# kikimo/tla-raft

Measured on AMD Instinct MI355X. Metric: distinct states/sec (whole node) + wall-time to exhaust, higher is better.
Workload: dtype u32

## Files before the change

tla-raft_amd/csrc/rmc_engine.hip:

```cpp
#include <hip/hip_runtime.h>
#include <hipcub/hipcub.hpp>

#include <algorithm>
#include <array>
#include <chrono>
#include <condition_variable>
#include <cstdio>
#include <cstdlib>
#include <cstring>
#include <memory>
#include <mutex>
#include <set>
#include <string>
#include <thread>
#include <vector>

#include <fcntl.h>
#include <sys/mman.h>
#include <unistd.h>

#include "rmc.h"
#include "rmc_kernels.h"
#include "rmc_plan.h"
#include "rmc_graph.h"
// ... 727 lines not shown
    void graph_level(Shard &s, uint64_t gid_cur, uint64_t n_par, uint64_t gid_nxt, uint64_t n_new, uint64_t bound_pos,
                     uint32_t bound_key, int kind) {
        try {
            graph_states(s, s.nxt_off, s.nbase(), n_new, gid_nxt);
            graph_edges(s, gid_cur, n_par, bound_pos, bound_key, kind);
        } catch (const Fail &e) {
            finished = true;
            status = e.code;
            throw;
        }
    }

    bool inited = false, finished = false;
    bool device_released = false;
    int status = RMC_OK;
    int depth = 0;
    uint64_t total_generated = 0, total_distinct = 0, queue_at_end = 0;
    int violated = -1;
    uint64_t err_ref = 0;
    uint32_t err_last_slot = KEY_NONE;
    std::vector<uint64_t> glevel;
    int L_shard = 0;
    std::vector<TraceStep> trace;
    double seconds = 0;

    KParams base(const Shard &s) const {
        KParams P{};
        P.d = U.d;
        P.E = cfg.max_election;
        P.R = cfg.max_restart;
        P.seeded = cfg.spec_variant == RMC_SPEC_SEEDED;
        P.quirks = (cfg.spec_variant == RMC_SPEC_SPLIT_BRAIN ? 1u : 0u) | (cfg.spec_variant == RMC_SPEC_COMMIT_PAST_LOG ? 2u : 0u);
        P.check_deadlock = cfg.check_deadlock;
        P.inv_mask = cfg.invariants;
        P.inv_order = inv_order;
        P.t.info = d_info;
        P.t.nat2id = d_nat2id;
        P.t.gmsg = d_gmsg;
        P.t.seeds = d_seeds;
        P.t.np = np;
        P.t.bmw = (uint32_t)((U.info.size() + 31) / 32);
        P.seen = s.seen();
        P.rcap = ~0ull;
        P.err = s.err;
        P.flags = s.flags;
        P.par = s.par;
        P.pslot = s.pslot;
        P.trace_base = s.tdev;
        return P;
    }

    void ring_params(const Shard &s, KParams &P) const {
        P.front = s.R;
        P.foff = s.cur_off;
        P.fbase = s.cur_wbase;
        P.rcap = s.rcap;
        P.next = s.R;
        P.noff = s.nxt_off;
        P.nbase = s.nbase();
    }

    KParams chunk_params(const Shard &s) const {
        KParams Q = base(s);
        ring_params(s, Q);
        Q.cnt = s.cnt; Q.fp = s.fp; Q.wpos = s.wpos; Q.wcnt = s.wcnt; Q.wacc = s.wacc; Q.pnm = s.pnm;
        Q.wposw = s.wposw; Q.bw = s.bw; Q.bg = s.bg; Q.boff = s.boff; Q.bww = s.bww; Q.boffw = s.boffw;
        Q.bn = s.bn; Q.boffn = s.boffn;
        Q.tickets = s.tickets; Q.ctick = s.ctick; Q.sum = s.sum;
        Q.score = s.score; Q.lslot = s.lslot; Q.ET = s.E; Q.hctx = s.hctx;
        return Q;
    }

    const int lookahead = env_int("RMC_LOOKAHEAD", 1, 0, 1);
    bool two_sets() const { return lookahead && !multi; }

    static uint32_t probe_dedup_entries() {
        const int v = env_int("RMC_PROBE_DEDUP", 1, 0, (int)PD_ENTRIES);
        if (v <= 1) return v ? PD_ENTRIES : 0u;
        uint32_t n = 2;
        while (2 * n <= (uint32_t)v) n *= 2;
        return n;
    }
    const uint32_t probe_dedup = probe_dedup_entries();
    const uint32_t probe_run = (uint32_t)env_int("RMC_PROBE_RUN", 0, 0, 64);
    const int probe_log = env_int("RMC_PROBE_DEDUP_LOG", 0, 0, 1);

    static constexpr unsigned ITEMS_MIN_BLOCKS = 2048;
    const int items_grid_env = env_int("RMC_ITEMS_GRID", 0, 0, 1 << 20);
    unsigned items_xgrid = 0, items_cgrid = 0;
    void size_items_grids(int cus) {
        int xb = 0, cb = 0;
        HIPCHK(ks.items_blocks(&xb, &cb));
        auto whole = [&](int per_cu) {
            const unsigned gen = (unsigned)(per_cu * cus);
            return gen ? (ITEMS_MIN_BLOCKS + gen - 1) / gen * gen : 0u;
        };
        items_xgrid = items_grid_env ? (unsigned)items_grid_env : whole(xb);
        items_cgrid = items_grid_env ? (unsigned)items_grid_env : whole(cb);
    }

    void swap_staging(Shard &s) {
        Staging &a = s.alt;
        std::swap(s.score, a.score); std::swap(s.hctx, a.hctx); std::swap(s.cnt, a.cnt); std::swap(s.pnm, a.pnm);
        std::swap(s.hcnt, a.hcnt); std::swap(s.hoff, a.hoff);
        std::swap(s.err, a.err); std::swap(s.sum, a.sum); std::swap(s.flags, a.flags);
        std::swap(s.xdone, a.done); std::swap(s.xt0, a.t0); std::swap(s.xt1, a.t1); std::swap(s.xtimed, a.timed);
        s.ocnt = reinterpret_cast<uint32_t *>(s.sum + SUM_OCNT);
    }
    static void alt_params(const Staging &a, KParams &Q) {
        Q.score = a.score; Q.hctx = a.hctx; Q.cnt = a.cnt; Q.pnm = a.pnm;
        Q.err = a.err; Q.sum = a.sum; Q.flags = a.flags;
    }
    void xwait() {
        if (xpending) HIPCHK(hipStreamSynchronize(xstream));
    }
    void drop_lookahead() {
        if (!xpending) return;
        xpending = false;
// ... 3762 lines not shown
```

tla-raft_amd/csrc/rmc_kernels.h:

```cpp
#pragma once
#include <hip/hip_runtime.h>
#include <stdint.h>

#include "rmc_spec.h"

namespace rmc {

struct Tables {
    const uint32_t *info;
    const uint16_t *nat2id;
    const ulonglong2 *gmsg;
    const uint64_t *seeds;
    int np;
    uint32_t bmw;
};

struct ESlot {
    unsigned long long x, y;
    unsigned long long k;
    unsigned long long pad;
};

struct Seen {
    ulonglong2 *T;
// ... 7 lines not shown
enum CtlStop : uint32_t { CTL_RUN = 0, CTL_DONE = 1, CTL_ERROR = 2, CTL_HOST = 3 };
struct LevelCtl {
    unsigned long long cur_n;
    unsigned long long gid_cur;
    unsigned long long T_count;
    unsigned long long Lmask;
    unsigned long long cur_wbase, cur_words;
    unsigned long long off_cap, rcap, trace_base, trace_cap, T_cap, chunk_parents, Lcap_max;
    uint32_t level;
    uint32_t epoch;
    uint32_t stop;
    uint32_t done_levels;
    uint32_t batch;
    uint32_t pad_;
};
struct LevelRec { unsigned long long expanded, generated, new_states, words, self_loops; };
constexpr int LREC_CAP = 1024;
struct HostLoop {
    uint32_t done;
    uint32_t stop;
    uint32_t pad_[2];
    LevelCtl ctl;
    LevelRec rec[LREC_CAP];
};
constexpr uint32_t WTILE = 1024;
constexpr uint32_t WTILES_MAX = 4096;
constexpr int SUM_WORDS = 7;
constexpr int SUM_INS = 9;
constexpr int SUM_INS_COMMIT = 10;
constexpr int SUM_NZ = 16;
constexpr int SUM_SELF = 17;
constexpr int SUM_HFP = 18;
constexpr uint32_t PD_ENTRIES = 512;
constexpr int PROBE_RUN = 2;
constexpr int SUM_OCNT = 20;
constexpr int SUM_PDROP = 56;
constexpr int SUM_SELF_STRIPE = 64, SELF_STRIDE = 16, SELF_STRIPES = 8;
constexpr int SUM_WORDS_TOTAL = 192;


struct KParams {
    Dims d;
    int E, R, seeded, check_deadlock;
    uint32_t inv_mask;
    uint32_t inv_order;
    Tables t;
    const uint32_t *front;
    const uint64_t *foff;
    uint64_t fbase, rcap;
    uint64_t p_begin, p_end;
    uint32_t *cnt;
    uint32_t *hcnt;
    uint32_t *hoff;
    const uint32_t *off;
    ulonglong2 *fp;
    const uint32_t *wflag;
    uint32_t *wpos;
    Seen seen;
    uint32_t *next;
    uint64_t *noff;
    uint64_t nbase;
    uint64_t next_wbase;
    uint64_t next_base;
    uint64_t *par;
    uint16_t *pslot;
    uint64_t trace_base;
    uint64_t gid_next_base;
    uint64_t gid_parent_base;
    unsigned long long *err;
    uint32_t *flags;
    int route;
    uint4 *xside;
    uint32_t *ocnt;
    uint32_t nown;
    ESlot *OT;
    uint64_t ot_mask, gblk;
    uint32_t ot_round, self;
    int split;
    uint32_t *hctx;
    uint32_t pdedup, prun;
    uint32_t quirks;
    uint4 *score;
    uint32_t *lslot;
    ESlot *ET;
    uint64_t Lmask;
    uint32_t epoch;
    uint32_t *wcnt;
    uint32_t *wacc;
    uint32_t *pnm;
    uint32_t *wposw;
    uint32_t *bw, *bg, *boff;
    uint32_t *bww, *boffw;
    uint32_t *bn, *boffn;
    uint32_t *plist;
    uint32_t *tickets;
    uint32_t *ctick;
    unsigned long long *sum;
    LevelCtl *ctl;
    LevelCtl *ctl_next;
    LevelRec *lrec;
    HostLoop *hloop;
    uint32_t done_levels;
    uint32_t *out_keys;
    uint32_t *out_count;
};

enum WalkEnd : uint32_t {
    WALK_DEPTH = 0,
    WALK_STUCK = 1,
    WALK_DEADLOCK = 2,
    WALK_ASSERT = 3,
    WALK_VIOLATION = 4,
    WALK_EVAL = 5,
// ... 108 lines not shown
```

tla-raft_amd/csrc/rmc_kernels.hip:

```cpp
#include <hip/hip_runtime.h>

#include <algorithm>

#include "rmc_kernels.h"

#ifdef RMC_PHASE_PROF
__device__ unsigned long long g_phase[16];
#define PHASE_DECL unsigned long long _acc[8] = {0, 0, 0, 0, 0, 0, 0, 0}; long long _tp = clock64();
#define PHASE(k) do { const long long _t = clock64(); _acc[k] += (unsigned long long)(_t - _tp); _tp = _t; } while (0)
#define PHASE_FLUSH_AT(b) do { if (threadIdx.x == 0) for (int _k = 0; _k < 8; _k++) atomicAdd(&g_phase[(b) + _k], _acc[_k]); } while (0)
#define PHASE_FLUSH PHASE_FLUSH_AT(0)
extern "C" int rmc_debug_phases(unsigned long long *out, int reset) {
    if (hipMemcpyFromSymbol(out, HIP_SYMBOL(g_phase), sizeof(unsigned long long) * 16) != hipSuccess) return -1;
    if (reset) {
        unsigned long long z[16] = {0};
        if (hipMemcpyToSymbol(HIP_SYMBOL(g_phase), z, sizeof(z)) != hipSuccess) return -1;
    }
    return 16;
}
#else
#define PHASE_DECL
#define PHASE(k) do {} while (0)
#define PHASE_FLUSH do {} while (0)
#define PHASE_FLUSH_AT(b) do {} while (0)
#endif

#ifndef RMC_N3_WAVES
#define RMC_N3_WAVES 4
#endif
#ifndef RMC_N3_COMMIT_WAVES
#define RMC_N3_COMMIT_WAVES 1
#endif
#ifndef RMC_GRID_PER_CU
#define RMC_GRID_PER_CU 32
#endif
#ifndef RMC_WIDE_WAVES
#define RMC_WIDE_WAVES 2
#endif

namespace rmc {

enum Mode { M_SINGLE = 3, M_FUSED = 4 };

template <int N>
__device__ __forceinline__ uint32_t sel(const uint32_t *a, int i) {
    uint32_t r = a[0];
#pragma unroll
    for (int k = 1; k < N; k++) r = (i == k) ? a[k] : r;
    return r;
}

__device__ __forceinline__ uint32_t rdlane(uint32_t v, int l) { return __builtin_amdgcn_readlane(v, l); }
__device__ __forceinline__ uint64_t rdlane64(uint64_t v, int l) {
    uint32_t lo = __builtin_amdgcn_readlane((uint32_t)v, l);
    uint32_t hi = __builtin_amdgcn_readlane((uint32_t)(v >> 32), l);
    return ((uint64_t)hi << 32) | lo;
}
// ... 1537 lines not shown
    return vf | (ct << 4) | (role << 8) | (ci << 12) | (ll << 16) | (s << 20);
}

template <int MCAP>
__device__ __forceinline__ bool ids_contain(const uint16_t *ids, uint32_t nm, uint32_t g) {
    uint32_t pos = 0;
#pragma unroll
    for (uint32_t st = (uint32_t)MCAP; st; st >>= 1)
        if (pos + st <= nm && (uint32_t)ids[pos + st - 1] < g) pos += st;
    return pos < nm && (uint32_t)ids[pos] == g;
}

template <int NADD>
struct RowSucc {
    uint32_t w0, lw, mirow, nirow, pend, misc;
    uint32_t key;
    uint32_t nadd;
    uint32_t add[NADD];
    uint32_t ainf[NADD];
    bool self;
};

template <int NADD>
__device__ __forceinline__ void row_stage(const RowSucc<NADD> &o, uint32_t nm, int sw4, uint4 *dst) {
    uint32_t a[4] = {0u, 0u, 0u, 0u};
#pragma unroll
    for (int k = 0; k < NADD; k++) a[k] = o.add[k];
    const uint32_t misc = (o.misc & ~0xFF0000u) | ((nm + o.nadd) << 16);
    dst[0] = make_uint4(o.w0, o.lw, o.mirow, o.nirow);
    dst[1] = make_uint4(o.pend, misc, o.key | (o.nadd << 16), a[0] | (a[1] << 16));
    if (sw4 > 2) dst[2] = make_uint4(a[2] | (a[3] << 16), 0u, 0u, 0u);
}

template <int N, int V, int MR, bool BFV>
__device__ __forceinline__ void item_msg(const KParams &P, const uint32_t *pc, const uint16_t *ids, uint32_t nm,
                                         uint32_t k, uint32_t m, uint32_t pid, RowSucc<Spec<N, V, MR>::NADD> &o,
                                         RowSucc<Spec<N, V, MR>::NADD> &ob, uint32_t &akey) {
    using Lo = Layout<N, V>;
    using S = Spec<N, V, MR>;
    const uint32_t s = mi_dst(m), typ = mi_type(m), mt = mi_term(m), src = mi_src(m);
    uint32_t vf = nib(pc[Lo::W_VF], s), ct = nib(pc[Lo::W_CT], s), role = nib(pc[Lo::W_ROLE], s);
    uint32_t ci = nib(pc[Lo::W_CI], s), ll = nib(pc[Lo::W_LL], s);
    const uint32_t lw = pc[Lo::W_LOG + s], mirow = pc[Lo::W_MI + s], nirow = pc[Lo::W_NI + s];
    const uint32_t pend = pc[Lo::W_PEND], misc = pc[Lo::W_MISC];
    o.key = KEY_NONE;
    o.nadd = 0;
    o.self = false;
#pragma unroll
    for (int a = 0; a < S::NADD; a++) o.add[a] = 0;
    o.lw = lw; o.mirow = mirow; o.nirow = nirow; o.pend = pend; o.misc = misc;
    o.w0 = row_w0(vf, ct, role, ci, ll, s);
    if (BFV) {
        ob = o;
        const bool up = mt > ct, step = mt == ct && typ == AREQ && role == CAN;
        if (up || step) {
            const uint32_t bct = up ? mt : ct, brole = role != FOL ? (uint32_t)FOL : role;
            const uint32_t bvf = (role != FOL && up) ? VF_NONE : vf;
            ob.w0 = row_w0(bvf, bct, brole, ci, ll, s);
            ob.key = slot_key(s, BF, k);
        }
    }
    if (mt > ct) {
        o.w0 = row_w0(VF_NONE, mt, FOL, ci, ll, s);
        o.key = slot_key(s, UT, k);
        return;
    }
// ... 18 lines not shown
    if (typ == AREQ && role == FOL) {
        const uint32_t pli = mi_x1(m), plt = mi_x2(m), lc = mi_x3(m), ent = mi_ent(m);
        const bool match = pli <= ll && plt == lw_term(lw, pli);
        if (match) {
            const uint32_t nl = pli + ent;
            const bool append_new = nl > ll;
            const uint32_t eb = mi_et(m) | (mi_ev(m) << 4);
            const bool truncated = nl <= ll && ent && lw_byte(lw, nl) != eb;
            const uint32_t mn = (lc < nl || (P.quirks & 2u)) ? lc : nl;
            const uint32_t nci = ci > mn ? ci : mn;
            uint32_t nll = ll;
            if (truncated || append_new) {
                const uint32_t keep = pli >= 2 ? (pli - 1) * 8 : 0;
                uint32_t nlw = keep >= 32 ? lw : (lw & ((1u << keep) - 1u));
                if (ent) nlw |= eb << (8 * (nl - 2));
                o.lw = nlw;
                nll = nl;
            }
            o.w0 = row_w0(vf, ct, role, nci, nll, s);
            const bool has = ids_contain<S::MCAP>(ids, nm, pid);
            if (!has) { o.add[0] = pid; o.nadd = 1; }
            o.ainf[0] = minfo(ARESP, s, src, mt, pli + ent, 1, 0, 0, 0, 0);
            o.self = has && !(truncated || append_new) && nci == ci;
            o.key = slot_key(s, FAE, k);
        } else {
            if (ids_contain<S::MCAP>(ids, nm, pid)) return;
            o.add[0] = pid; o.nadd = 1;
            o.ainf[0] = minfo(ARESP, s, src, mt, pli, 0, 0, 0, 0, 0);
            o.key = slot_key(s, FRE, k);
        }
        return;
    }
    if (typ == ARESP && role == LEA) {
        const uint32_t pb = s * N + src;
        if (!((pend >> pb) & 1u)) return;
        const uint32_t pli = mi_x1(m);
        const uint32_t mi = nib(mirow, src), ni = nib(nirow, src);
        uint32_t nmi = mirow, nni = nirow;
        if (mi_x2(m)) {
            if (!(mi < pli)) return;
            nmi = setnib(mirow, src, pli);
            nni = setnib(nirow, src, pli + 1);
        } else {
            if (!(pli + 1 == ni)) return;
            if (!(pli > mi)) return;
            nni = setnib(nirow, src, pli);
        }
        o.mirow = nmi;
        o.nirow = nni;
        o.pend = pend & ~(1u << pb);
        o.key = slot_key(s, HAR, k);
    }
}

template <int N, int V>
__device__ __forceinline__ uint32_t item_msg_nat(const KParams &P, const uint32_t *pc, uint32_t m) {
    using Lo = Layout<N, V>;
    const uint32_t s = mi_dst(m), typ = mi_type(m), mt = mi_term(m), src = mi_src(m);
    if (mt != nib(pc[Lo::W_CT], s) || nib(pc[Lo::W_ROLE], s) != FOL) return NAT_NONE;
    if (typ == VREQ) return nat_vresp(P.d, s, src, mt);
    if (typ != AREQ) return NAT_NONE;
    const uint32_t ll = nib(pc[Lo::W_LL], s), lw = pc[Lo::W_LOG + s];
    const uint32_t pli = mi_x1(m), plt = mi_x2(m), ent = mi_ent(m);
    const bool match = pli <= ll && plt == lw_term(lw, pli);
    return match ? nat_aresp(P.d, s, src, mt, pli + ent, 1) : nat_aresp(P.d, s, src, mt, pli, 0);
}

template <int N, int V, int MR>
__device__ __forceinline__ void item_slot(const KParams &P, const uint32_t *pc, const uint16_t *ids, uint32_t nm,
                                          uint32_t vp, uint32_t s, uint32_t t, RowSucc<Spec<N, V, MR>::NADD> &o) {
    using Lo = Layout<N, V>;
    using S = Spec<N, V, MR>;
    const uint32_t vf = nib(pc[Lo::W_VF], s), ct = nib(pc[Lo::W_CT], s), role = nib(pc[Lo::W_ROLE], s);
    const uint32_t ci = nib(pc[Lo::W_CI], s), ll = nib(pc[Lo::W_LL], s);
    const uint32_t lw = pc[Lo::W_LOG + s], mirow = pc[Lo::W_MI + s], nirow = pc[Lo::W_NI + s];
    const uint32_t pend = pc[Lo::W_PEND], misc = pc[Lo::W_MISC];
    o.key = KEY_NONE;
    o.nadd = 0;
    o.self = false;
#pragma unroll
    for (int a = 0; a < S::NADD; a++) o.add[a] = 0;
    o.lw = lw; o.mirow = mirow; o.nirow = nirow; o.pend = pend; o.misc = misc;
    o.w0 = row_w0(vf, ct, role, ci, ll, s);
    if (t == 0) {
        const uint32_t ec = misc & 15u;
        if (!((int)ec < P.E) || !(role == FOL || role == CAN)) return;
        const uint32_t term = ct + 1, llt = lw_term(lw, ll);
        uint32_t sid[N - 1];
#pragma unroll
        for (int i = 0; i < N - 1; i++) {
            const uint32_t p = (uint32_t)i < s ? (uint32_t)i : (uint32_t)i + 1u;
            sid[i] = (uint32_t)P.t.nat2id[nat_vreq(P.d, s, p, term, ll, llt)];
        }
        uint32_t na = 0;
#pragma unroll
        for (int i = 0; i < N - 1; i++) {
            if (!ids_contain<S::MCAP>(ids, nm, sid[i])) {
                const uint32_t p = (uint32_t)i < s ? (uint32_t)i : (uint32_t)i + 1u;
                const uint32_t inf = minfo(VREQ, s, p, term, ll, llt, 0, 0, 0, 0);
#pragma unroll
                for (int a = 0; a < S::NADD; a++) {
                    o.add[a] = ((uint32_t)a == na) ? sid[i] : o.add[a];
                    o.ainf[a] = ((uint32_t)a == na) ? inf : o.ainf[a];
                }
                na++;
            }
        }
        o.nadd = na;
        o.w0 = row_w0(s, term, CAN, ci, ll, s);
        o.misc = (misc & ~15u) | (ec + 1);
        o.key = slot_key(s, BC, 0);
        return;
    }
    if (t == 1) {
        if (role != CAN) return;
        if (!(vp + 1 >= ((P.quirks & 1u) ? 1u : (uint32_t)(N / 2 + 1)))) return;
        uint32_t mr = 0, nr = 0;
#pragma unroll
        for (int u = 0; u < N; u++) {
            mr = setnib(mr, u, (uint32_t)u != s ? 1u : ll);
            nr = setnib(nr, u, ll + 1);
        }
        o.mirow = mr;
        o.nirow = nr;
        o.pend = pend & ~(((1u << N) - 1u) << (s * N));
        o.w0 = row_w0(vf, ct, LEA, ci, ll, s);
        o.key = slot_key(s, BL, 0);
        return;
    }
    if (role != LEA) return;
    if (t < 2 + (uint32_t)V) {
        const uint32_t v = t - 2;
        if ((misc >> (8 + v)) & 1u) return;
        o.misc = misc | (1u << (8 + v));
        o.lw = lw | ((ct | (v << 4)) << (8 * (ll + 1 - 2)));
        o.mirow = setnib(mirow, s, ll + 1);
        o.w0 = row_w0(vf, ct, role, ci, ll + 1, s);
        o.key = slot_key(s, CR, v);
        return;
    }
    if (t < 2 + (uint32_t)V + (N - 1)) {
        const uint32_t q = t - 2 - V;
        const uint32_t dst = q < s ? q : q + 1;
        const uint32_t ni = nib(nirow, dst);
        if (!(ni <= ll + 1)) return;
        const uint32_t pb = s * N + dst;
        if ((pend >> pb) & 1u) return;
        const uint32_t pli = ni - 1, plt = lw_term(lw, pli);
        const uint32_t ent = ni <= ll ? 1u : 0u;
        const uint32_t eb = ent ? lw_byte(lw, ni) : 0u;
        const uint32_t id = P.t.nat2id[nat_areq(P.d, s, dst, ct, pli, plt, ent, eb & 15u, eb >> 4, ci)];
        if (ids_contain<S::MCAP>(ids, nm, id)) return;
        o.pend = pend | (1u << pb);
        o.add[0] = id;
        o.ainf[0] = minfo(AREQ, s, dst, ct, pli, plt, ci, ent, eb & 15u, eb >> 4);
        o.nadd = 1;
        o.key = slot_key(s, LAE, dst);
        return;
    }
    if (t == 2 + (uint32_t)V + (N - 1)) {
        const uint32_t thr = P.seeded ? (uint32_t)N : (uint32_t)(N / 2 + 1);
        const uint32_t med = median_row<N>(mirow, thr);
        if (!(med > ci)) return;
        o.w0 = row_w0(vf, ct, role, med, ll, s);
        o.key = slot_key(s, LCC, 0);
        return;
    }
    {
        const uint32_t rc = (misc >> 4) & 15u;
        if (!((int)rc < P.R)) return;
        o.w0 = row_w0(vf, ct, FOL, ci, ll, s);
        o.misc = (misc & ~0xF0u) | ((rc + 1) << 4);
        o.key = slot_key(s, RS, 0);
    }
}

template <int N, int V>
__device__ __forceinline__ uint32_t slot_range(uint32_t role, uint32_t ec, uint32_t rc, int E, int R) {
    constexpr uint32_t SPS = 4 + V + (N - 1);
    if (role == LEA) return 2u | ((SPS - 2u - ((int)rc < R ? 0u : 1u)) << 4);
    const uint32_t bc = (int)ec < E ? 1u : 0u;
    if (role == CAN) return (bc ? 0u : 1u) | ((bc + 1u) << 4);
    return bc << 4;
}

template <int N, int V, int MR, bool BFV>
constexpr int items_waves() {
#ifdef RMC_ITEMS_WAVES
    return RMC_ITEMS_WAVES;
#else
    return (MR == 1 && !(BFV && N == 3 && V >= 2)) ? 5 : 0;
#endif
}
enum ItemClass : uint32_t {
    IC_UT = 0,
    IC_UT2,
    IC_RV,
    IC_AE,
    IC_HAR,
    IC_BC, IC_BL, IC_CR, IC_LAE, IC_LCC, IC_RS,
    IC_N,
    IC_DEAD = 0xFF
};
__device__ __forceinline__ uint32_t msg_class(uint32_t m, uint32_t ct, uint32_t role) {
    const uint32_t mt = mi_term(m), typ = mi_type(m);
    if (mt > ct) return IC_UT;
    if (mt < ct) return IC_DEAD;
    if (typ == AREQ) return role != FOL ? IC_UT2 : IC_AE;
    if (typ == VREQ) return role == FOL ? IC_RV : IC_DEAD;
    if (typ == ARESP) return role == LEA ? IC_HAR : IC_DEAD;
    return IC_DEAD;
}
template <int N, int V>
__device__ __forceinline__ uint32_t slot_class(uint32_t t) {
    return t == 0 ? IC_BC : t == 1 ? IC_BL : t < 2 + (uint32_t)V ? IC_CR : t < 2 + (uint32_t)V + (N - 1) ? IC_LAE
         : t == 2 + (uint32_t)V + (N - 1) ? IC_LCC : IC_RS;
}

template <int N, int V, int MR, bool BFV, bool FUSE, int PB>
__global__ __launch_bounds__((items_threads<N, V, MR, FUSE>()), FUSE ? ((N <= 3 && !BFV) ? RMC_FUSED_WAVES : 0) : (items_waves<N, V, MR, BFV>())) void k_expand_items(KParams P) {
    using S = Spec<N, V, MR>;
    using Lo = Layout<N, V>;
    constexpr int NT = items_threads<N, V, MR, FUSE>();
    static_assert(PB >= 2 && PB <= 64 && (PB & (PB - 1)) == 0, "parents per batch: a power of two, a lane of wave 0 each");
    constexpr int CCW = S::CCW, RECW = S::RECW_MAX, NW = Lo::NW, NWP = (NW + 3) / 4 * 4;
    constexpr int MX = S::MAXS + (BFV ? S::MCAP : 0);
    constexpr int NCI = BFV ? 2 : 1;
    constexpr int NPR = N * (N - 1);
    constexpr int CTXW = ctx_words<N, V>(), CC = ((CCW + 3) / 4) * 4;
    constexpr int RC = FUSE ? 1 : 4;
    static_assert(S::MCAP + N * S::SLOTS_PER_SERVER <= NT, "a parent's items fit one evaluation round");
    static_assert(S::MCAP <= 128 && PB <= 64, "item codes: parent << 8 | slot bit << 7 | message index or s << 4 | t");
    __shared__ uint32_t sRec[PB * RECW];
    __shared__ uint32_t sCore[PB * NWP];
    __shared__ uint8_t sMI[PB * S::MCAP];
    __shared__ uint8_t sMJ[PB * S::MCAP];
    __shared__ uint32_t sInf[FUSE ? PB * S::MCAP : 1];
    __shared__ uint32_t sVp[PB * N];
    __shared__ uint32_t sOff[PB];
    __shared__ uint32_t sItm[PB + 1], sMsc[PB + 1];
    __shared__ uint32_t sLive[PB];
    __shared__ unsigned long long sSlot[PB];
    __shared__ uint32_t sCnt[PB], sAk[PB];
    __shared__ uint32_t sHo[FUSE ? 1 : PB];
    __shared__ uint32_t sAlloc;
    __shared__ uint32_t sSelf[PB];
    __shared__ uint32_t sCc[IC_N];
    constexpr int UM = FUSE ? 0 : 2 * PB * NPR * 8, UQ = IC_N * NT * 2 + NT * NCI * 2;
    __shared__ __attribute__((aligned(16))) unsigned char sU[UM > UQ ? UM : UQ];
    __shared__ unsigned long long sMh[FUSE ? 2 * PB * NPR : 1];
    __shared__ uint64_t sK[2][FUSE ? N * N : 1];
    unsigned long long *sM0 = FUSE ? sMh : reinterpret_cast<unsigned long long *>(sU), *sM1 = sM0 + PB * NPR;
    uint16_t *sQ = reinterpret_cast<uint16_t *>(sU);
    uint16_t *sKey = sQ + IC_N * NT;
    __shared__ uint32_t sSpan;
    __shared__ uint32_t sSelfN;
    __shared__ uint32_t sHfp;
    const int tid = threadIdx.x;
    if (tid == 0) {
        sSelfN = 0u;
        sHfp = 0u;
    }
    if constexpr (FUSE) {
        if (!level_args(P)) return;
        if (P.hloop && blockIdx.x == 0 && tid == 0)
// ... 27 lines not shown
            const uint64_t f0 = P.foff[P.p_begin + b0];
            const uint64_t start = ring_wrap(P.fbase + f0, P.rcap);
            const uint32_t span = sSpan;
            for (uint32_t w0 = (uint32_t)tid; w0 < span; w0 += RC * NT) {
                uint32_t v[RC];
#pragma unroll
                for (int k = 0; k < RC; k++)
                    if (w0 + k * NT < span) v[k] = ring_word(P.front, start, w0 + k * NT, P.rcap);
#pragma unroll
                for (int k = 0; k < RC; k++)
                    if (w0 + k * NT < span) sRec[w0 + k * NT] = v[k];
            }
        }
        __syncthreads();
        PHASE(0);
        if (tid < 64) {
            uint32_t nmj = 0;
            if ((uint32_t)tid < nb) {
                const uint32_t *rec = sRec + sOff[tid];
                uint32_t pk[CCW], c[NW];
#pragma unroll
                for (int k = 0; k < CCW; k++) pk[k] = rec[k];
                decode_core<N, V>(pk, c);
                nmj = (c[Lo::W_MISC] >> 16) & 0xFFu;
                if (nmj > (uint32_t)S::MCAP) {
                    atomicOr(&P.flags[0], 1u);
                    nmj = S::MCAP;
                    c[Lo::W_MISC] = (c[Lo::W_MISC] & ~0xFF0000u) | (nmj << 16);
                }
#pragma unroll
                for (int w = 0; w < NW; w++) sCore[tid * NWP + w] = c[w];
                const uint32_t ec = c[Lo::W_MISC] & 15u, rc = (c[Lo::W_MISC] >> 4) & 15u;
                unsigned long long sl = 0;
#pragma unroll
                for (int s = 0; s < N; s++)
                    sl |= (unsigned long long)slot_range<N, V>(nib(c[Lo::W_ROLE], s), ec, rc, P.E, P.R) << (8 * s);
                sSlot[tid] = sl;
#pragma unroll
                for (int s = 0; s < N; s++) sVp[tid * N + s] = 0u;
#pragma unroll
                for (int k = 0; k < NPR; k++) { sM0[tid * NPR + k] = 0ull; sM1[tid * NPR + k] = 0ull; }
                sCnt[tid] = 0u;
                sSelf[tid] = 0u;
                sAk[tid] = KEY_NONE;
                sLive[tid] = 0u;
            }
            uint32_t tm;
            const uint32_t xm = wave_excl_scan(nmj, tid, &tm);
            if ((uint32_t)tid < nb) sMsc[tid] = xm;
            if (tid == 0) sMsc[nb] = tm;
            for (uint32_t k = 0; k < nmj; k++) sMJ[xm + k] = (uint8_t)tid;
        }
        __syncthreads();
        PHASE(1);
        const uint32_t tmsg = sMsc[nb];
        for (uint32_t m = (uint32_t)tid; m < tmsg; m += NT) {
            const uint32_t j = sMJ[m];
            const uint32_t k = m - sMsc[j];
            const uint32_t id = reinterpret_cast<const uint16_t *>(sRec + sOff[j] + CCW)[k];
            const uint32_t inf = P.t.info[id];
            const ulonglong2 g = P.t.gmsg[id];
            const uint32_t src = mi_src(inf), dst = mi_dst(inf);
            const int pi = pair_index(N, (int)src, (int)dst);
            atomicAdd(&sM0[j * NPR + pi], (unsigned long long)g.x);
            atomicAdd(&sM1[j * NPR + pi], (unsigned long long)g.y);
            const uint32_t *pc = sCore + j * NWP;
            const uint32_t ct = nib(pc[Lo::W_CT], dst);
            if (mi_type(inf) == VRESP && mi_term(inf) == ct) atomicAdd(&sVp[j * N + dst], 1u);
            const uint32_t c = msg_class(inf, ct, nib(pc[Lo::W_ROLE], dst));
            sMI[m] = (uint8_t)(c == IC_DEAD ? 15u : c);
            if constexpr (FUSE) sInf[m] = inf;
            if (c != IC_DEAD) atomicAdd(&sLive[j], 1u);
        }
        __syncthreads();
        PHASE(2);
        for (uint32_t w = (uint32_t)tid; !FUSE && w < nb * (uint32_t)CTXW; w += NT) {
            const uint32_t j = w / CTXW, k = w % CTXW;
            uint32_t v = 0u;
            if (k < (uint32_t)CC) {
                v = k < (uint32_t)CCW ? sRec[sOff[j] + k] : 0u;
            } else {
                const uint32_t pi = (k - CC) >> 2, part = k & 3u;
                const unsigned long long mm = (part >> 1) ? sM1[j * NPR + pi] : sM0[j * NPR + pi];
                v = (part & 1u) ? (uint32_t)(mm >> 32) : (uint32_t)mm;
            }
            P.hctx[(b0 + j) * (uint64_t)CTXW + k] = v;
        }
        if (tid < 64) {
            uint32_t ni = 0;
            if ((uint32_t)tid < nb) {
                const unsigned long long sl = sSlot[tid];
                ni = sLive[tid];
#pragma unroll
                for (int u = 0; u < N; u++) ni += (uint32_t)(sl >> (8 * u + 4)) & 15u;
            }
            uint32_t ti;
            const uint32_t xi = wave_excl_scan(ni, tid, &ti);
            if ((uint32_t)tid < nb) sItm[tid] = xi;
            if (tid == 0) sItm[nb] = ti;
        }
        if (tid < IC_N) sCc[tid] = 0u;
        __syncthreads();
        PHASE(3);
        for (uint32_t a = 0; a < nb;) {
            const uint32_t ibase = sItm[a];
            uint32_t b = a;
#pragma unroll
            for (uint32_t st = PB; st; st >>= 1) b = (b + st <= nb && sItm[b + st] <= ibase + NT) ? b + st : b;
            b = b > a ? b : a + 1;
            const uint32_t nI = sItm[b] - ibase < (uint32_t)NT ? sItm[b] - ibase : (uint32_t)NT;
            for (uint32_t m = sMsc[a] + (uint32_t)tid; m < sMsc[b]; m += NT) {
                const uint32_t c = sMI[m];
                if (c == 15u) continue;
                const uint32_t j = sMJ[m];
                sQ[c * NT + atomicAdd(&sCc[c], 1u)] = (uint16_t)((j << 8) | (m - sMsc[j]));
            }
            for (uint32_t q = (uint32_t)tid; q < (b - a) * (uint32_t)N; q += NT) {
                const uint32_t j = a + q / N, u = q % N;
                const uint32_t rg = (uint32_t)(sSlot[j] >> (8 * u)) & 0xFFu, n = rg >> 4, t0 = rg & 15u;
                uint32_t pos[S::SLOTS_PER_SERVER];
#pragma unroll
                for (uint32_t r = 0; r < (uint32_t)S::SLOTS_PER_SERVER; r++)
                    if (r < n) pos[r] = atomicAdd(&sCc[slot_class<N, V>(t0 + r)], 1u);
#pragma unroll
                for (uint32_t r = 0; r < (uint32_t)S::SLOTS_PER_SERVER; r++)
                    if (r < n) sQ[slot_class<N, V>(t0 + r) * NT + pos[r]] = (uint16_t)((j << 8) | 0x80u | (u << 4) | (t0 + r));
            }
            __syncthreads();
            PHASE(7);
            RowSucc<S::NADD> o, ob;
            o.key = KEY_NONE;
            ob.key = KEY_NONE;
            uint32_t j = 0, nmj = 0;
            if ((uint32_t)tid < nI) {
                uint32_t pre = 0, code = 0;
#pragma unroll
                for (uint32_t c = 0; c < IC_N; c++) {
                    const uint32_t n = sCc[c], t = (uint32_t)tid - pre;
                    if (t < n) code = sQ[c * NT + t];
                    pre += n;
                }
                j = code >> 8;
                const uint32_t *pc = sCore + j * NWP;
                const uint16_t *ids = reinterpret_cast<const uint16_t *>(sRec + sOff[j] + CCW);
                nmj = (pc[Lo::W_MISC] >> 16) & 0xFFu;
                uint32_t akey = KEY_NONE;
                if (!(code & 0x80u)) {
                    const uint32_t k = code & 0x7Fu;
                    const uint32_t inf = FUSE ? sInf[sMsc[j] + k] : P.t.info[ids[k]];
                    const uint32_t nat = item_msg_nat<N, V>(P, pc, inf);
                    const uint32_t pid = nat != NAT_NONE ? (uint32_t)P.t.nat2id[nat] : 0u;
                    item_msg<N, V, MR, BFV>(P, pc, ids, nmj, k, inf, pid, o, ob, akey);
                } else {
                    const uint32_t s = (code >> 4) & 7u, t = code & 15u;
                    item_slot<N, V, MR>(P, pc, ids, nmj, sVp[j * N + s], s, t, o);
                }
                if (akey != KEY_NONE) atomicMin(&sAk[j], akey);
                const uint32_t kb = (sItm[j] - ibase) * NCI;
                if (!FUSE && o.key != KEY_NONE && o.self && P.hcnt) atomicAdd(&sSelf[j], 1u);
// ... 1639 lines not shown
}

template <class K>
static hipError_t resident_blocks(K kernel, int threads, int *blocks) {
    int api = 0;
    const hipError_t e = hipOccupancyMaxActiveBlocksPerMultiprocessor(&api, kernel, threads, 0);
    if (e != hipSuccess) return e;
    constexpr int SGPR_MAX = 106;
    const int waves = std::min(8, 800 / ((SGPR_MAX + 15) / 16 * 16 + 16));
    const int per_simd = (threads + 255) / 256;
    *blocks = std::max(1, std::min(api, waves / per_simd));
    return hipSuccess;
}

template <int N, int V, int MR, bool BFV = false>
struct Launch {
    static constexpr int MX = Spec<N, V, MR>::MAXS + (BFV ? Spec<N, V, MR>::MCAP : 0);
    static size_t bm_bytes(const KParams &P) { return (size_t)P.t.bmw * 4; }
    static void single(const KParams &P, hipStream_t s) {
        hipLaunchKernelGGL((k_expand<N, V, MR, M_SINGLE, BFV>), dim3(1), dim3(64), bm_bytes(P), s, P);
    }
    static void fused(const KParams &P, hipStream_t s) {
        if (!P.route) {
            const uint64_t nbat = (P.p_end - P.p_begin + XF_PARENTS - 1) / XF_PARENTS;
            hipLaunchKernelGGL((k_expand_items<N, V, MR, BFV, true, XF_PARENTS>), dim3((unsigned)(nbat < 8192 ? (nbat ? nbat : 1) : 8192)),
                               dim3(XB_THREADS), 0, s, P);
            return;
        }
        hipLaunchKernelGGL((k_expand<N, V, MR, M_FUSED, BFV>), dim3(grid_for(P.p_end - P.p_begin)), dim3(64),
                           bm_bytes(P), s, P);
    }
    static void split(const KParams &P, unsigned grid, hipStream_t s) {
        const uint64_t nbat = (P.p_end - P.p_begin + XB_PARENTS - 1) / XB_PARENTS;
        hipLaunchKernelGGL((k_expand_items<N, V, MR, BFV, false, XB_PARENTS>), dim3(items_grid(nbat, grid)),
                           dim3(items_threads<N, V, MR, false>()), 0, s, P);
    }
    static unsigned items_grid(uint64_t nbat, unsigned grid) {
        const uint64_t cap = grid ? grid : 2048u;
        return (unsigned)(nbat < cap ? (nbat ? nbat : 1) : cap);
    }
    static hipError_t items_blocks(int *expand, int *commit) {
        *commit = 0;
        hipError_t e = resident_blocks(k_expand_items<N, V, MR, BFV, false, XB_PARENTS>, items_threads<N, V, MR, false>(), expand);
        if constexpr (MX <= XB_THREADS) {
            if (e == hipSuccess) e = resident_blocks(k_commit_items<N, V, MR, MX, false, 64, false>, XB_THREADS, commit);
        }
        return e;
    }
    static void hash_probe(const KParams &P, uint64_t np, hipStream_t s) {
        KParams Q = P;
        const uint64_t fit = np / (256ull * 1024ull);
        Q.prun = P.route ? 1u : P.prun ? P.prun : (uint32_t)(fit < 1 ? 1 : fit < (uint64_t)PROBE_RUN ? fit : (uint64_t)PROBE_RUN);
        const uint64_t per = 256ull * Q.prun;
        const uint64_t blocks = (np + per - 1) / per;
        hipLaunchKernelGGL((k_hash_probe<N, V, MR, MX>), dim3(blocks ? (unsigned)(blocks < 16384ull ? blocks : 16384ull) : 1u),
                           dim3(256), 0, s, Q);
    }
    static void insert(const KParams &P, uint64_t np, hipStream_t s) {
        const uint64_t blocks = (np + 255) / 256;
        hipLaunchKernelGGL((k_insert_winners<MX>), dim3(blocks ? (unsigned)(blocks < 16384ull ? blocks : 16384ull) : 1u),
                           dim3(256), 0, s, P);
    }
    static void wincount(const KParams &P, uint64_t np, hipStream_t s) {
        const uint64_t tiles = (np + WTILE - 1) / WTILE;
        hipLaunchKernelGGL((k_wincount<N, V, MR>), dim3(tiles ? (unsigned)tiles : 1u), dim3(1024), 0, s, P);
    }
    static void commit(const KParams &P, hipStream_t s) {
        if constexpr (MX <= XB_THREADS) {
            if (!P.route && !P.split && !P.plist) {
                const uint64_t nbat = (P.p_end - P.p_begin + XC_PARENTS - 1) / XC_PARENTS;
                hipLaunchKernelGGL((k_commit_items<N, V, MR, MX, true, XC_PARENTS>),
                                   dim3((unsigned)(nbat < 8192 ? (nbat ? nbat : 1) : 8192)), dim3(XB_THREADS), 0, s, P);
                return;
            }
        }
        hipLaunchKernelGGL((k_commit<N, V, MR, BFV>), dim3(grid_for(P.p_end - P.p_begin)), dim3(64), 0, s, P);
// ... 384 lines not shown
```

Measured before the change: 1.124 billion.

## Prefilter disabled action slots and dead append-responses before item evaluation

Adds a prefilter mode to the split item-expansion kernel. Enabling guards for every server action slot, and the append-response guard, are now evaluated per parent up front, so the slot ranges become exact bitmasks and dead items are never enqueued or evaluated. The goal is less wasted per-item work and fewer items in the evaluation rounds. In exchange it adds a per-wave guard pass with shared atomics, an extra barrier, and a second kernel instantiation; the resident-block count is taken as the minimum across both variants.

```diff
diff --git a/tla-raft_amd/csrc/rmc_engine.hip b/tla-raft_amd/csrc/rmc_engine.hip
--- a/tla-raft_amd/csrc/rmc_engine.hip
+++ b/tla-raft_amd/csrc/rmc_engine.hip
@@ -783,6 +783,7 @@
         P.seeded = cfg.spec_variant == RMC_SPEC_SEEDED;
         P.quirks = (cfg.spec_variant == RMC_SPEC_SPLIT_BRAIN ? 1u : 0u) | (cfg.spec_variant == RMC_SPEC_COMMIT_PAST_LOG ? 2u : 0u);
         P.check_deadlock = cfg.check_deadlock;
+        P.prefilter = item_prefilter;
         P.inv_mask = cfg.invariants;
         P.inv_order = inv_order;
         P.t.info = d_info;
@@ -835,6 +836,8 @@
     const uint32_t probe_dedup = probe_dedup_entries();
     const uint32_t probe_run = (uint32_t)env_int("RMC_PROBE_RUN", 0, 0, 64);
     const int probe_log = env_int("RMC_PROBE_DEDUP_LOG", 0, 0, 1);
+
+    const uint32_t item_prefilter = (uint32_t)env_int("RMC_ITEM_PREFILTER", RMC_ITEM_PREFILTER_DEFAULT, 0, 3) & 1u;
 
     static constexpr unsigned ITEMS_MIN_BLOCKS = 2048;
     const int items_grid_env = env_int("RMC_ITEMS_GRID", 0, 0, 1 << 20);
diff --git a/tla-raft_amd/csrc/rmc_kernels.h b/tla-raft_amd/csrc/rmc_kernels.h
--- a/tla-raft_amd/csrc/rmc_kernels.h
+++ b/tla-raft_amd/csrc/rmc_kernels.h
@@ -63,6 +63,7 @@
 constexpr int SUM_SELF = 17;
 constexpr int SUM_HFP = 18;
 constexpr uint32_t PD_ENTRIES = 512;
+constexpr int RMC_ITEM_PREFILTER_DEFAULT = 1;
 constexpr int PROBE_RUN = 2;
 constexpr int SUM_OCNT = 20;
 constexpr int SUM_PDROP = 56;
@@ -110,6 +111,7 @@
     int split;
     uint32_t *hctx;
     uint32_t pdedup, prun;
+    uint32_t prefilter;
     uint32_t quirks;
     uint4 *score;
     uint32_t *lslot;
diff --git a/tla-raft_amd/csrc/rmc_kernels.hip b/tla-raft_amd/csrc/rmc_kernels.hip
--- a/tla-raft_amd/csrc/rmc_kernels.hip
+++ b/tla-raft_amd/csrc/rmc_kernels.hip
@@ -6,10 +6,11 @@
 
 #ifdef RMC_PHASE_PROF
 __device__ unsigned long long g_phase[16];
-#define PHASE_DECL unsigned long long _acc[8] = {0, 0, 0, 0, 0, 0, 0, 0}; long long _tp = clock64();
+#define PHASE_DECL unsigned long long _acc[8] = {0, 0, 0, 0, 0, 0, 0, 0}, _cn[3] = {0, 0, 0}; (void)_cn; long long _tp = clock64();
 #define PHASE(k) do { const long long _t = clock64(); _acc[k] += (unsigned long long)(_t - _tp); _tp = _t; } while (0)
 #define PHASE_FLUSH_AT(b) do { if (threadIdx.x == 0) for (int _k = 0; _k < 8; _k++) atomicAdd(&g_phase[(b) + _k], _acc[_k]); } while (0)
-#define PHASE_FLUSH PHASE_FLUSH_AT(0)
+#define PHASE_COUNT(i, n) do { _cn[i] += (unsigned long long)(n); } while (0)
+#define PHASE_FLUSH do { PHASE_FLUSH_AT(0); if (threadIdx.x == 0) { atomicAdd(&g_phase[11], _cn[0]); atomicAdd(&g_phase[14], _cn[1]); atomicAdd(&g_phase[15], _cn[2]); } } while (0)
 extern "C" int rmc_debug_phases(unsigned long long *out, int reset) {
     if (hipMemcpyFromSymbol(out, HIP_SYMBOL(g_phase), sizeof(unsigned long long) * 16) != hipSuccess) return -1;
     if (reset) {
@@ -23,6 +24,7 @@
 #define PHASE(k) do {} while (0)
 #define PHASE_FLUSH do {} while (0)
 #define PHASE_FLUSH_AT(b) do {} while (0)
+#define PHASE_COUNT(i, n) do {} while (0)
 #endif
 
 #ifndef RMC_N3_WAVES
@@ -1626,6 +1628,14 @@
     if (sw4 > 2) dst[2] = make_uint4(a[2] | (a[3] << 16), 0u, 0u, 0u);
 }
 
+template <int N>
+__device__ __forceinline__ bool har_guard(uint32_t pend, uint32_t mirow, uint32_t nirow, uint32_t s, uint32_t m) {
+    const uint32_t src = mi_src(m), pli = mi_x1(m);
+    if (!((pend >> (s * N + src)) & 1u)) return false;
+    const uint32_t mi = nib(mirow, src), ni = nib(nirow, src);
+    return mi_x2(m) ? mi < pli : (pli + 1 == ni && pli > mi);
+}
+
 template <int N, int V, int MR, bool BFV>
 __device__ __forceinline__ void item_msg(const KParams &P, const uint32_t *pc, const uint16_t *ids, uint32_t nm,
                                          uint32_t k, uint32_t m, uint32_t pid, RowSucc<Spec<N, V, MR>::NADD> &o,
@@ -1710,18 +1720,13 @@
         return;
     }
     if (typ == ARESP && role == LEA) {
-        const uint32_t pb = s * N + src;
-        if (!((pend >> pb) & 1u)) return;
-        const uint32_t pli = mi_x1(m);
-        const uint32_t mi = nib(mirow, src), ni = nib(nirow, src);
+        if (!har_guard<N>(pend, mirow, nirow, s, m)) return;
+        const uint32_t pb = s * N + src, pli = mi_x1(m);
         uint32_t nmi = mirow, nni = nirow;
         if (mi_x2(m)) {
-            if (!(mi < pli)) return;
             nmi = setnib(mirow, src, pli);
             nni = setnib(nirow, src, pli + 1);
         } else {
-            if (!(pli + 1 == ni)) return;
-            if (!(pli > mi)) return;
             nni = setnib(nirow, src, pli);
         }
         o.mirow = nmi;
@@ -1742,6 +1747,24 @@
     const uint32_t pli = mi_x1(m), plt = mi_x2(m), ent = mi_ent(m);
     const bool match = pli <= ll && plt == lw_term(lw, pli);
     return match ? nat_aresp(P.d, s, src, mt, pli + ent, 1) : nat_aresp(P.d, s, src, mt, pli, 0);
+}
+
+template <int N, int V>
+__device__ __forceinline__ bool slot_guard(const KParams &P, const uint32_t *pc, uint32_t vp, uint32_t s, uint32_t t) {
+    using Lo = Layout<N, V>;
+    const uint32_t role = nib(pc[Lo::W_ROLE], s), misc = pc[Lo::W_MISC];
+    if (t == 0) return (int)(misc & 15u) < P.E && (role == FOL || role == CAN);
+    if (t == 1)
+        return role == CAN && vp + 1 >= ((P.quirks & 1u) ? 1u : (uint32_t)(N / 2 + 1));
+    if (role != LEA) return false;
+    if (t < 2 + (uint32_t)V) return !((misc >> (8 + (t - 2))) & 1u);
+    if (t < 2 + (uint32_t)V + (N - 1)) {
+        const uint32_t q = t - 2 - V, dst = q < s ? q : q + 1;
+        return nib(pc[Lo::W_NI + s], dst) <= nib(pc[Lo::W_LL], s) + 1 && !((pc[Lo::W_PEND] >> (s * N + dst)) & 1u);
+    }
+    if (t == 2 + (uint32_t)V + (N - 1))
+        return median_row<N>(pc[Lo::W_MI + s], P.seeded ? (uint32_t)N : (uint32_t)(N / 2 + 1)) > nib(pc[Lo::W_CI], s);
+    return (int)((misc >> 4) & 15u) < P.R;
 }
 
 template <int N, int V, int MR>
@@ -1760,9 +1783,9 @@
     for (int a = 0; a < S::NADD; a++) o.add[a] = 0;
     o.lw = lw; o.mirow = mirow; o.nirow = nirow; o.pend = pend; o.misc = misc;
     o.w0 = row_w0(vf, ct, role, ci, ll, s);
+    if (!slot_guard<N, V>(P, pc, vp, s, t)) return;
     if (t == 0) {
         const uint32_t ec = misc & 15u;
-        if (!((int)ec < P.E) || !(role == FOL || role == CAN)) return;
         const uint32_t term = ct + 1, llt = lw_term(lw, ll);
         uint32_t sid[N - 1];
 #pragma unroll
@@ -1791,8 +1814,6 @@
         return;
     }
     if (t == 1) {
-        if (role != CAN) return;
-        if (!(vp + 1 >= ((P.quirks & 1u) ? 1u : (uint32_t)(N / 2 + 1)))) return;
         uint32_t mr = 0, nr = 0;
 #pragma unroll
         for (int u = 0; u < N; u++) {
@@ -1806,10 +1827,8 @@
         o.key = slot_key(s, BL, 0);
         return;
     }
-    if (role != LEA) return;
     if (t < 2 + (uint32_t)V) {
         const uint32_t v = t - 2;
-        if ((misc >> (8 + v)) & 1u) return;
         o.misc = misc | (1u << (8 + v));
         o.lw = lw | ((ct | (v << 4)) << (8 * (ll + 1 - 2)));
         o.mirow = setnib(mirow, s, ll + 1);
@@ -1821,9 +1840,7 @@
         const uint32_t q = t - 2 - V;
         const uint32_t dst = q < s ? q : q + 1;
         const uint32_t ni = nib(nirow, dst);
-        if (!(ni <= ll + 1)) return;
         const uint32_t pb = s * N + dst;
-        if ((pend >> pb) & 1u) return;
         const uint32_t pli = ni - 1, plt = lw_term(lw, pli);
         const uint32_t ent = ni <= ll ? 1u : 0u;
         const uint32_t eb = ent ? lw_byte(lw, ni) : 0u;
@@ -1839,14 +1856,12 @@
     if (t == 2 + (uint32_t)V + (N - 1)) {
         const uint32_t thr = P.seeded ? (uint32_t)N : (uint32_t)(N / 2 + 1);
         const uint32_t med = median_row<N>(mirow, thr);
-        if (!(med > ci)) return;
         o.w0 = row_w0(vf, ct, role, med, ll, s);
         o.key = slot_key(s, LCC, 0);
         return;
     }
     {
         const uint32_t rc = (misc >> 4) & 15u;
-        if (!((int)rc < P.R)) return;
         o.w0 = row_w0(vf, ct, FOL, ci, ll, s);
         o.misc = (misc & ~0xF0u) | ((rc + 1) << 4);
         o.key = slot_key(s, RS, 0);
@@ -1895,7 +1910,7 @@
          : t == 2 + (uint32_t)V + (N - 1) ? IC_LCC : IC_RS;
 }
 
-template <int N, int V, int MR, bool BFV, bool FUSE, int PB>
+template <int N, int V, int MR, bool BFV, bool FUSE, int PB, int PF = 0>
 __global__ __launch_bounds__((items_threads<N, V, MR, FUSE>()), FUSE ? ((N <= 3 && !BFV) ? RMC_FUSED_WAVES : 0) : (items_waves<N, V, MR, BFV>())) void k_expand_items(KParams P) {
     using S = Spec<N, V, MR>;
     using Lo = Layout<N, V>;
@@ -1909,6 +1924,10 @@
     constexpr int RC = FUSE ? 1 : 4;
     static_assert(S::MCAP + N * S::SLOTS_PER_SERVER <= NT, "a parent's items fit one evaluation round");
     static_assert(S::MCAP <= 128 && PB <= 64, "item codes: parent << 8 | slot bit << 7 | message index or s << 4 | t");
+    constexpr uint32_t SLOT_BITS = 12;
+    static_assert(S::SLOTS_PER_SERVER <= (int)SLOT_BITS && N * SLOT_BITS <= 64, "a server's slots: a bitmask in its part of sSlot's word");
+    static_assert(NT >= 64 && NT % 64 == 0, "the slot masks: a whole wave per server, lane j of it the batch's parent j");
+    constexpr uint32_t pf = FUSE ? 0u : (uint32_t)PF;
     __shared__ uint32_t sRec[PB * RECW];
     __shared__ uint32_t sCore[PB * NWP];
     __shared__ uint8_t sMI[PB * S::MCAP];
@@ -2002,9 +2021,13 @@
                 for (int w = 0; w < NW; w++) sCore[tid * NWP + w] = c[w];
                 const uint32_t ec = c[Lo::W_MISC] & 15u, rc = (c[Lo::W_MISC] >> 4) & 15u;
                 unsigned long long sl = 0;
-#pragma unroll
-                for (int s = 0; s < N; s++)
-                    sl |= (unsigned long long)slot_range<N, V>(nib(c[Lo::W_ROLE], s), ec, rc, P.E, P.R) << (8 * s);
+                if (!(pf & 1u)) {
+#pragma unroll
+                    for (int s = 0; s < N; s++) {
+                        const uint32_t rg = slot_range<N, V>(nib(c[Lo::W_ROLE], s), ec, rc, P.E, P.R);
+                        sl |= (unsigned long long)(((1u << (rg >> 4)) - 1u) << (rg & 15u)) << (SLOT_BITS * s);
+                    }
+                }
                 sSlot[tid] = sl;
 #pragma unroll
                 for (int s = 0; s < N; s++) sVp[tid * N + s] = 0u;
@@ -2037,7 +2060,12 @@
             const uint32_t *pc = sCore + j * NWP;
             const uint32_t ct = nib(pc[Lo::W_CT], dst);
             if (mi_type(inf) == VRESP && mi_term(inf) == ct) atomicAdd(&sVp[j * N + dst], 1u);
-            const uint32_t c = msg_class(inf, ct, nib(pc[Lo::W_ROLE], dst));
+            uint32_t c = msg_class(inf, ct, nib(pc[Lo::W_ROLE], dst));
+            if constexpr (!FUSE) {
+                if ((pf & 1u) && c == IC_HAR &&
+                    !har_guard<N>(pc[Lo::W_PEND], pc[Lo::W_MI + dst], pc[Lo::W_NI + dst], dst, inf))
+                    c = IC_DEAD;
+            }
             sMI[m] = (uint8_t)(c == IC_DEAD ? 15u : c);
             if constexpr (FUSE) sInf[m] = inf;
             if (c != IC_DEAD) atomicAdd(&sLive[j], 1u);
@@ -2056,13 +2084,23 @@
             }
             P.hctx[(b0 + j) * (uint64_t)CTXW + k] = v;
         }
+        if (!FUSE && (pf & 1u)) {
+            const uint32_t j = (uint32_t)tid & 63u;
+            for (uint32_t u = __builtin_amdgcn_readfirstlane((uint32_t)tid >> 6); u < (uint32_t)N && j < nb; u += NT >> 6) {
+                const uint32_t *pc = sCore + j * NWP;
+                const uint32_t vp = sVp[j * N + u];
+                uint32_t mk = 0;
+#pragma unroll
+                for (uint32_t t = 0; t < (uint32_t)S::SLOTS_PER_SERVER; t++)
+                    mk |= slot_guard<N, V>(P, pc, vp, u, t) ? 1u << t : 0u;
+                if (mk) atomicOr(&sSlot[j], (unsigned long long)mk << (SLOT_BITS * u));
+            }
+            __syncthreads();
+        }
         if (tid < 64) {
             uint32_t ni = 0;
             if ((uint32_t)tid < nb) {
-                const unsigned long long sl = sSlot[tid];
-                ni = sLive[tid];
-#pragma unroll
-                for (int u = 0; u < N; u++) ni += (uint32_t)(sl >> (8 * u + 4)) & 15u;
+                ni = sLive[tid] + (uint32_t)__popcll(sSlot[tid]);
             }
             uint32_t ti;
             const uint32_t xi = wave_excl_scan(ni, tid, &ti);
@@ -2072,7 +2110,10 @@
         if (tid < IC_N) sCc[tid] = 0u;
         __syncthreads();
         PHASE(3);
+        PHASE_COUNT(0, 1u);
+        PHASE_COUNT(2, sItm[nb]);
         for (uint32_t a = 0; a < nb;) {
+            PHASE_COUNT(1, 1u);
             const uint32_t ibase = sItm[a];
             uint32_t b = a;
 #pragma unroll
@@ -2087,14 +2128,14 @@
             }
             for (uint32_t q = (uint32_t)tid; q < (b - a) * (uint32_t)N; q += NT) {
                 const uint32_t j = a + q / N, u = q % N;
-                const uint32_t rg = (uint32_t)(sSlot[j] >> (8 * u)) & 0xFFu, n = rg >> 4, t0 = rg & 15u;
+                const uint32_t mk = (uint32_t)(sSlot[j] >> (SLOT_BITS * u)) & ((1u << SLOT_BITS) - 1u);
                 uint32_t pos[S::SLOTS_PER_SERVER];
 #pragma unroll
-                for (uint32_t r = 0; r < (uint32_t)S::SLOTS_PER_SERVER; r++)
-                    if (r < n) pos[r] = atomicAdd(&sCc[slot_class<N, V>(t0 + r)], 1u);
-#pragma unroll
-                for (uint32_t r = 0; r < (uint32_t)S::SLOTS_PER_SERVER; r++)
-                    if (r < n) sQ[slot_class<N, V>(t0 + r) * NT + pos[r]] = (uint16_t)((j << 8) | 0x80u | (u << 4) | (t0 + r));
+                for (uint32_t t = 0; t < (uint32_t)S::SLOTS_PER_SERVER; t++)
+                    if ((mk >> t) & 1u) pos[t] = atomicAdd(&sCc[slot_class<N, V>(t)], 1u);
+#pragma unroll
+                for (uint32_t t = 0; t < (uint32_t)S::SLOTS_PER_SERVER; t++)
+                    if ((mk >> t) & 1u) sQ[slot_class<N, V>(t) * NT + pos[t]] = (uint16_t)((j << 8) | 0x80u | (u << 4) | t);
             }
             __syncthreads();
             PHASE(7);
@@ -3800,8 +3841,9 @@
     }
     static void split(const KParams &P, unsigned grid, hipStream_t s) {
         const uint64_t nbat = (P.p_end - P.p_begin + XB_PARENTS - 1) / XB_PARENTS;
-        hipLaunchKernelGGL((k_expand_items<N, V, MR, BFV, false, XB_PARENTS>), dim3(items_grid(nbat, grid)),
-                           dim3(items_threads<N, V, MR, false>()), 0, s, P);
+        auto k = P.prefilter ? k_expand_items<N, V, MR, BFV, false, XB_PARENTS, 1>
+                             : k_expand_items<N, V, MR, BFV, false, XB_PARENTS, 0>;
+        hipLaunchKernelGGL(k, dim3(items_grid(nbat, grid)), dim3(items_threads<N, V, MR, false>()), 0, s, P);
     }
     static unsigned items_grid(uint64_t nbat, unsigned grid) {
         const uint64_t cap = grid ? grid : 2048u;
@@ -3809,7 +3851,10 @@
     }
     static hipError_t items_blocks(int *expand, int *commit) {
         *commit = 0;
-        hipError_t e = resident_blocks(k_expand_items<N, V, MR, BFV, false, XB_PARENTS>, items_threads<N, V, MR, false>(), expand);
+        int x1 = 0;
+        hipError_t e = resident_blocks(k_expand_items<N, V, MR, BFV, false, XB_PARENTS, 0>, items_threads<N, V, MR, false>(), expand);
+        if (e == hipSuccess) e = resident_blocks(k_expand_items<N, V, MR, BFV, false, XB_PARENTS, 1>, items_threads<N, V, MR, false>(), &x1);
+        if (e == hipSuccess) *expand = std::min(*expand, x1);
         if constexpr (MX <= XB_THREADS) {
             if (e == hipSuccess) e = resident_blocks(k_commit_items<N, V, MR, MX, false, 64, false>, XB_THREADS, commit);
         }
```

After: 1.186 billion, median of 6. +5.5%, better.
